# akloetgen/PARA-suite

Measured on AMD Instinct MI355X. Metric: aligned reads/sec (10Mx50bp PAR-CLIP vs hg19-size genome) on MI355X; SAM bit-exact vs own CPU restatement (parity unpinned), higher is better.
Workload: dtype u64

## Files before the change

### para-suite_amd/csrc/ps_core.h

```cpp
#pragma once
#include "ps_types.h"

namespace ps {

PS_HD uint32_t ps_popc(uint32_t x)
{
#ifdef __HIP_DEVICE_COMPILE__
    return (uint32_t)__popc(x);
#else
    return (uint32_t)__builtin_popcount(x);
#endif
}
PS_HD uint32_t pfx_mask32(int ns)
{
    return ns >= 32 ? 0xFFFFFFFFu : (ns <= 0 ? 0u : ((1u << ns) - 1u));
}

struct Blk { uint32_t x[16]; };

#ifdef __HIP_DEVICE_COMPILE__
#define PS_AS_GLOBAL(T, p) ((const __attribute__((address_space(1))) T *)(p))
#define PS_AS_GLOBAL_W(T, p) ((__attribute__((address_space(1))) T *)(p))
typedef uint32_t ps_u32x4 __attribute__((ext_vector_type(4)));
typedef uint32_t ps_u32x2 __attribute__((ext_vector_type(2)));
// ... 111 lines not shown
    blk_count4(xk, need_k ? ok_ + 1 : 0, ck);
    if (!need_k) { ck[0] = ck[1] = ck[2] = ck[3] = 0; }
    ++st.pairs;
    if (need_k && !other) ++st.same;
}
PS_HD void occ_pair1(const IndexView &ix, bwtint k, bwtint l, int c, uint32_t &ok, uint32_t &ol, LaneStats &st)
{
    int ol_ = 0, ok_ = 0;
    const uint32_t bl = blk_of(row_to_stored(ix.primary, l), ol_);
    uint32_t bk = bl;
    bool need_k = k != 0;
    if (need_k) bk = blk_of(row_to_stored(ix.primary, k - 1), ok_);
    Blk xl, xk;
    load_blk(ix.blocks, bl, xl);
    bool other = need_k && bk != bl;
    if (other) load_blk(ix.blocks, bk, xk);
    ol = blk_count1(xl, ol_ + 1, c);
    if (!need_k) ok = 0;
    else if (other) ok = blk_count1(xk, ok_ + 1, c);
    else ok = blk_count1(xl, ok_ + 1, c);
    ++st.pairs;
    if (need_k && !other) ++st.same;
}

PS_HD int read_base(const uint32_t *bases, const uint32_t *nmask, int n_reads, int r, int j)
{
    uint32_t w = bases[(size_t)(j >> 4) * n_reads + r];
    uint32_t m = nmask[(size_t)(j >> 5) * n_reads + r];
    return ((m >> (j & 31)) & 1u) ? 4 : (int)((w >> (2 * (j & 15))) & 3u);
}

PS_HD uint8_t cw_pack(int bid, bool eq) { return (uint8_t)((bid > 127 ? 127 : bid) | (eq ? 0x80 : 0)); }

struct WChain { bwtint k, l; int bid; uint32_t prev_w; };
PS_HD void wchain_init(const IndexView &ix, WChain &c) { c.k = 0; c.l = ix.seq_len; c.bid = 0; c.prev_w = 0xFFFFFFFFu; }
PS_HD void wchain_step(const IndexView &ix, WChain &c, int base, uint32_t &w_out, uint8_t &cw_out, bool first, LaneStats &st)
{
    if (base < 4) {
        uint32_t ok, ol;
        occ_pair1(ix, c.k, c.l, base, ok, ol, st);
        const bwtint l2 = L2_of(ix, base);
        c.k = l2 + ok + 1;
        c.l = l2 + ol;
    }
    if (c.k > c.l || base > 3) { c.k = 0; c.l = ix.seq_len; ++c.bid; }
    uint32_t w = width32(c.k, c.l);
    w_out = w;
    cw_out = cw_pack(c.bid, !first && w == c.prev_w);
    c.prev_w = w;
}

static const int PS_POP_TRIES = 1;
enum { M_FETCH = 0, M_POP = 1, M_EXACT = 2, M_EXPAND = 3, M_EXIT = 4, M_HIT = 5,
       M_GROW = 6 };

struct BtLane {
    int r, mode;
    bwtint k, l;
    int i, score, units, n_mm, n_gapo, n_gape, n_ins, n_del, state, ldp;
    bool have_cur;
    int best_score, max_units, n_aln, n_stack, status;
    unsigned long long best_cnt;
    unsigned long long bm0, bm1;
    uint32_t bump, free_head, iters0;
    uint32_t rn0, rn1;
    int len;
    uint32_t n_phantom;
    uint32_t cap;
    LaneStats st;
};

PS_HD int lm_ncw(int len) { return (len + 1 + 3) >> 2; }
PS_HD int lm_ncsw(int seed_len) { return seed_len > 0 ? (seed_len + 1 + 3) >> 2 : 0; }
PS_HD bool lm_nmask_in_regs(int len) { return len <= 64; }
PS_HD int lm_heads_off(int len, int seed_len) { return 4 * (lm_ncw(len) + lm_ncsw(seed_len) + ((len + 15) >> 4) + (lm_nmask_in_regs(len) ? 0 : ((len + 31) >> 5))); }
PS_HD int lm_bytes(int len, int seed_len, int n_buckets, bool wide)
{
    int n = lm_heads_off(len, seed_len) + (wide ? 0 : 2 * n_buckets);
    n = (n + 3) & ~3;
    if (((n >> 2) & 1) == 0) n += 4;
    return n;
}

static const int PS_JUMP_SLOT_WORDS = 8, PS_JUMP_MAX_LEVELS = 14;
PS_HD uint32_t jump_level_off(int d) { return 0x55555555u & ((1u << (2 * d)) - 1u); }
PS_HD size_t jump_words(int levels) { return (size_t)jump_level_off(levels) * PS_JUMP_SLOT_WORDS; }
PS_HD int jump_levels_for(bwtint seq_len) { int k = 0; while (k < PS_JUMP_MAX_LEVELS && (seq_len >> (2 * k)) >= 48) ++k; return k; }

static const int PS_CHASE_MIN2 = 16;
struct BtHot {
    const OccBlock *blocks; bwtint primary;
    const uint32_t *jump; uint32_t jump_levels;
    uint32_t skip_levels;
    uint32_t L2lo[4], L2hi;
    uint32_t s_pk[5], u_pk[5];
    uint32_t p0, p1, p2, p3;
    uint32_t inv_c_min, max_entries, pool_cap, n_reads, big_cap;
    uint32_t c_min;
    uint32_t chase;
    PS_HD int len() const { return (int)(p0 & 0xffu); }
    PS_HD int seed_len() const { return (int)((p0 >> 8) & 0xffu); }
    PS_HD int indel_end_skip() const { return (int)((p0 >> 16) & 0xffu); }
    PS_HD int max_del_occ() const { return (int)(p0 >> 24); }
    PS_HD int max_gapo() const { return (int)(p1 & 0xfu); }
    PS_HD int max_gape() const { return (int)((p1 >> 4) & 0xfu); }
    PS_HD bool mode_gape() const { return ((p1 >> 8) & 1u) != 0; }
    PS_HD bool use_seed() const { return ((p1 >> 9) & 1u) != 0; }
    PS_HD bool profile() const { return ((p1 >> 10) & 1u) != 0; }
    PS_HD bool has_big() const { return ((p1 >> 11) & 1u) != 0; }
    PS_HD int seed_units() const { return (int)((p1 >> 12) & 0xfffu); }
    PS_HD int u_tight() const { return (int)(p1 >> 24); }
    PS_HD int s_gapo_ins() const { return (int)(p2 & 0xffu); }
    PS_HD int s_gape() const { return (int)((p2 >> 8) & 0xffu); }
    PS_HD int s_gapo_del() const { return (int)((p2 >> 16) & 0xffu); }
    PS_HD int s_stop() const { return (int)(p2 >> 24); }
    PS_HD int u_gapo_ins() const { return (int)(p3 & 0xffu); }
    PS_HD int u_gape() const { return (int)((p3 >> 8) & 0xffu); }
    PS_HD int u_gapo_del() const { return (int)((p3 >> 16) & 0xffu); }
    PS_HD int n_buckets() const { return (int)(p3 >> 24); }
    PS_HD bwtint L2(int c) const
// ... 426 lines not shown
```

### para-suite_amd/csrc/ps_effort.hip

```cpp
#include <hip/hip_runtime.h>
#include "ps_core.h"
#include <stdexcept>
#include "ps_kernels.h"
#include "ps_budget.h"

namespace ps {

struct EChain {
    bwtint k, l;
    uint32_t cost_lo, cost_hi;
    int piece;
    int n_rs;
    int cl_n, cl_last;
    uint32_t cl_lo, cl_hi;
};
__device__ __forceinline__ void echain_restart(const EffortArgs &a, EChain &c, bool lo_half)
{
    c.k = 0; c.l = a.ix.seq_len; c.piece = 0; c.cl_n = 0; ++c.n_rs;
    if (lo_half) c.cost_lo += (uint32_t)a.c_restart; else c.cost_hi += (uint32_t)a.c_restart;
}
__device__ __forceinline__ void echain_step(const EffortArgs &a, EChain &c, int sym, uint32_t cw, int pos, bool lo_half, LaneStats &st)
{
    uint32_t ck[4], cl[4];
    occ_pair4(a.ix.blocks, a.ix.primary, c.k, c.l, ck, cl, st);
    if (sym < 4) {
        const uint32_t ok = sel4(ck, sym), ol = sel4(cl, sym);
        if (ok < ol) { const bwtint b = L2_of(a.ix, sym); c.k = b + ok + 1; c.l = b + ol; ++c.piece; return; }
    }
    int best = -1; uint32_t best_cost = 0xffu;
    if (c.l - c.k < (bwtint)a.w_pin) {
#pragma unroll
        for (int t = 0; t < 4; ++t) {
            const uint32_t ct = (cw >> (8 * t)) & 0xffu;
            if (t != sym && ck[t] < cl[t] && ct < best_cost) { best = t; best_cost = ct; }
        }
    }
    if (best < 0) { echain_restart(a, c, lo_half); return; }
    const int d = pos > c.cl_last ? pos - c.cl_last : c.cl_last - pos;
    if (c.cl_n > 0 && d <= 4) ++c.cl_n; else { c.cl_n = 1; c.cl_lo = c.cost_lo; c.cl_hi = c.cost_hi; }
    c.cl_last = pos;
    if (lo_half) c.cost_lo += best_cost; else c.cost_hi += best_cost;
    if (c.cl_n >= 3) {
        c.k = 0; c.l = a.ix.seq_len; c.piece = 0; c.cl_n = 0; ++c.n_rs;
        return;
    }
    const bwtint b = L2_of(a.ix, best);
    c.k = b + sel4(ck, best) + 1; c.l = b + sel4(cl, best); ++c.piece;
}

__global__ void __launch_bounds__(256, 8) k_effort(EffortArgs a)
{
    const int lane = threadIdx.x & 63;
    const bool is_b = lane >= 32;
    const int wave = (int)((blockIdx.x * blockDim.x + threadIdx.x) >> 6), n_waves = (int)((gridDim.x * blockDim.x) >> 6);
    LaneStats st = {0, 0, 0, 0, 0, 0, 0, 0};
    for (int r = wave * 32 + (lane & 31); r < a.n_reads; r += n_waves * 32) {
        const int len = a.lens ? a.lens[r] : a.len, half = len >> 1;
        EChain C = {0, a.ix.seq_len, 0, 0, 0, 0, 0, 0, 0, 0};
        uint32_t bw = 0, mw = 0;
#pragma unroll 1
        for (int i = 0; i < len; ++i) {
            const int j = is_b ? i : len - 1 - i;
            if (i == 0 || (j & 15) == (is_b ? 0 : 15)) bw = a.bases[(size_t)(j >> 4) * a.n_reads + opaque_lane(r)];
            if (i == 0 || (j & 31) == (is_b ? 0 : 31)) mw = a.nmask[(size_t)(j >> 5) * a.n_reads + opaque_lane(r)];
            const int bs = ((mw >> (j & 31)) & 1u) ? 4 : (int)((bw >> (2 * (j & 15))) & 3u);
            const int sc = bs > 3 ? 4 : 3 - bs;
            const uint32_t cws = cost_word(a.s_pk, sc);
            const uint32_t cw = is_b ? cws : __builtin_bswap32(cws);
            echain_step(a, C, is_b ? sc : bs, cw, j, j < half, st);
        }
        const uint32_t mine = C.cost_lo + C.cost_hi;
        const uint32_t tb = (uint32_t)__shfl((int)mine, lane | 32, 64), ta = mine;
        const int b_rs = __shfl(C.n_rs, lane | 32, 64), a_rs = C.n_rs;
        if (!is_b) {
            const uint32_t e = a_rs == 0 ? (b_rs == 0 && tb < ta ? tb : ta) : (b_rs == 0 ? tb : (ta > tb ? ta : tb));
            a.est[r] = (uint8_t)(e > 255u ? 255u : e);
            if (a.est_ab) a.est_ab[r] = (uint16_t)((ta > 127u ? 127u : ta) | (a_rs ? 0x80u : 0u) | ((tb > 127u ? 127u : tb) << 8) | (b_rs ? 0x8000u : 0u));
        }
    }
}

template <int G>
__global__ void __launch_bounds__(256) k_effort_model(EffortModelArgs a)
{
    const int lane = threadIdx.x & 63, u = lane & (G - 1);
    const int per_wave = 64 / G;
    const long long wave = ((long long)blockIdx.x * blockDim.x + threadIdx.x) >> 6, n_waves = ((long long)gridDim.x * blockDim.x) >> 6;
    for (long long r0 = wave * per_wave + lane / G; r0 < a.n_reads; r0 += n_waves * per_wave) {
        const int r = (int)r0;
        const int len = a.lens ? a.lens[r] : a.len;
        const int own = (a.lens && a.units_by_len) ? (int)a.units_by_len[len] : a.max_units;
        int B = (int)a.est[r] + a.u_tight;
        if (B > own) B = own;
        float w = u == 0 ? 1.f : 0.f;
        float tot = 0.f, phi_rows = a.rows;
        const int depth = len < a.depth ? len : a.depth;
        const int rem = B - u;
        const int m = rem >= 0 ? (int)(((uint32_t)rem * a.inv_c_min) >> 16) : -1;
        const int srem = a.seed_units - u;
        const bool seed_ok = srem > 0 && (int)(((uint32_t)srem * a.inv_c_min) >> 16) >= 1;
        uint32_t info = 0;
        if (u < depth) {
// ... 74 lines not shown
```

### para-suite_amd/csrc/ps_kernels.h

```cpp
#pragma once
#include <hip/hip_runtime.h>
#include "ps_types.h"
#include "ps_budget.h"

namespace ps {

static const int PS_MAX_CIGAR = 16;

struct WidthArgs {
    IndexView ix;
    int n_reads, len, seed_len, use_seed;
    const int32_t *lens;
    const uint32_t *bases; const uint32_t *nmask;
    uint32_t *w; uint32_t *cwb; uint32_t *cswb;
    KStats *stats;
};

struct EffortArgs {
    IndexView ix;
    int n_reads, len;
    const int32_t *lens;
    const uint32_t *bases; const uint32_t *nmask;
    uint32_t s_pk[5];
    int c_restart;
    uint32_t w_pin;
    uint8_t *est;
    uint16_t *est_ab;
};

struct EffortModelArgs {
    int n_reads, len;
    const int32_t *lens; const uint8_t *units_by_len;
    const uint32_t *bases; const uint32_t *nmask; const uint32_t *cwb;
    const uint8_t *est;
    uint32_t s_pk[5]; uint32_t inv_c_min;
    int max_units, u_tight, seed_units, use_seed, seed_len;
    int max_gapo, indel_end_skip, u_gapo_ins, u_gapo_del;
    int depth;
    float rows;
    int log_scale;
    uint8_t *key; float *pred;
};

struct RefineItem { int32_t read; bwtint rb; int32_t ref_shift; int32_t strand; };
struct RefineArgs {
    IndexView ix;
    int n_items, len, n_reads;
    const int32_t *lens;
    const uint32_t *bases; const uint32_t *nmask;
    const RefineItem *items;
    uint32_t *cigar; int32_t *n_cigar;
    uint8_t *zbuf; size_t z_per_block;
    int32_t *hebuf; size_t he_per_block;
// ... 34 lines not shown
```

### para-suite_amd/csrc/ps_kernels.hip

```cpp
#include <hip/hip_runtime.h>
#include <algorithm>
#include <cstdlib>
#include <stdexcept>
#include <string>
#include "ps_core.h"
#include "ps_narrow.h"
#include "ps_kernels.h"

namespace ps {

static const int PS_Q_CHUNK = 64;
#ifndef PS_BT_WAVES
#define PS_BT_WAVES 4
#endif

__device__ __forceinline__ unsigned long long wave_sum(unsigned long long v)
{
    for (int o = 32; o > 0; o >>= 1) v += __shfl_xor(v, o, 64);
    return v;
}
__device__ __forceinline__ void flush_stats(KStats *ks, const LaneStats &st)
{
    if (!ks) return;
    unsigned long long v[8] = {st.pairs, st.same, st.nodes, st.pushes, st.pops, st.lf, st.iters, st.exact};
    unsigned long long *dst = reinterpret_cast<unsigned long long *>(ks);
#pragma unroll
    for (int j = 0; j < 8; ++j) {
        unsigned long long s = wave_sum(v[j]);
        if ((threadIdx.x & 63) == 0 && s) atomicAdd(dst + j, s);
    }
}

__global__ void __launch_bounds__(256, 8) k_width(WidthArgs a)
{
    const int roles = a.use_seed ? 2 : 1;
    const bool seed_role = roles == 2 && (blockIdx.x & 1) != 0;
    const int stride = (gridDim.x / roles) * blockDim.x;
    LaneStats st = {0, 0, 0, 0, 0, 0, 0, 0};
    for (int r = (blockIdx.x / roles) * blockDim.x + threadIdx.x; r < a.n_reads; r += stride) {
        WChain C;
        wchain_init(a.ix, C);
        const int len = a.lens ? a.lens[r] : a.len, seed_len = a.seed_len;
        const bool seeded = a.use_seed && len > seed_len;
        uint32_t bw = 0, mw = 0;
        uint32_t cww = 0;
        if (!seed_role) {
#pragma unroll 1
            for (int i = 0; i < len; ++i) {
                int j = len - 1 - i;
                if (i == 0 || (j & 15) == 15) bw = a.bases[(size_t)(j >> 4) * a.n_reads + opaque_lane(r)];
                if (i == 0 || (j & 31) == 31) mw = a.nmask[(size_t)(j >> 5) * a.n_reads + opaque_lane(r)];
                int base = ((mw >> (j & 31)) & 1u) ? 4 : (int)((bw >> (2 * (j & 15))) & 3u);
                uint32_t wv; uint8_t cb;
                wchain_step(a.ix, C, base, wv, cb, i == 0, st);
                a.w[(size_t)i * a.n_reads + opaque_lane(r)] = wv;
                cww |= (uint32_t)cb << (8 * (i & 3));
                if ((i & 3) == 3) { a.cwb[(size_t)(i >> 2) * a.n_reads + opaque_lane(r)] = cww; cww = 0; }
            }
            a.w[(size_t)len * a.n_reads + opaque_lane(r)] = 0;
            cww |= (uint32_t)cw_pack(C.bid + 1, false) << (8 * (len & 3));
            a.cwb[(size_t)(len >> 2) * a.n_reads + opaque_lane(r)] = cww;
        } else if (seeded) {
#pragma unroll 1
            for (int i = 0; i < seed_len; ++i) {
                int js = seed_len - 1 - i;
                if (i == 0 || (js & 15) == 15) bw = a.bases[(size_t)(js >> 4) * a.n_reads + opaque_lane(r)];
                if (i == 0 || (js & 31) == 31) mw = a.nmask[(size_t)(js >> 5) * a.n_reads + opaque_lane(r)];
                int sbase = ((mw >> (js & 31)) & 1u) ? 4 : (int)((bw >> (2 * (js & 15))) & 3u);
                uint32_t swv; uint8_t scb;
                wchain_step(a.ix, C, sbase, swv, scb, i == 0, st);
                cww |= (uint32_t)scb << (8 * (i & 3));
                if ((i & 3) == 3) { a.cswb[(size_t)(i >> 2) * a.n_reads + opaque_lane(r)] = cww; cww = 0; }
            }
            cww |= (uint32_t)cw_pack(C.bid + 1, false) << (8 * (seed_len & 3));
            a.cswb[(size_t)(seed_len >> 2) * a.n_reads + opaque_lane(r)] = cww;
        } else if (a.use_seed) {
            for (int p = 0; p <= (seed_len >> 2); ++p) a.cswb[(size_t)p * a.n_reads + opaque_lane(r)] = 0u;
        }
    }
    flush_stats(a.stats, st);
}

__device__ __forceinline__ uint32_t pin32(uint32_t v) { return (uint32_t)__builtin_amdgcn_readfirstlane((int)v); }
__device__ __forceinline__ unsigned long long pin64(unsigned long long v)
{
    return (unsigned long long)pin32((uint32_t)v) | ((unsigned long long)pin32((uint32_t)(v >> 32)) << 32);
}
__device__ __forceinline__ void pin_hot(BtHot &h, const BtHot &k)
{
    h.blocks = reinterpret_cast<const OccBlock *>(pin64(reinterpret_cast<unsigned long long>(k.blocks)));
    h.primary = pin64(k.primary);
    h.jump = reinterpret_cast<const uint32_t *>(pin64(reinterpret_cast<unsigned long long>(k.jump))); h.jump_levels = pin32(k.jump_levels); h.skip_levels = pin32(k.skip_levels);
#pragma unroll
    for (int c = 0; c < 4; ++c) h.L2lo[c] = pin32(k.L2lo[c]);
    h.L2hi = pin32(k.L2hi);
#pragma unroll
    for (int c = 0; c < 5; ++c) { h.s_pk[c] = pin32(k.s_pk[c]); h.u_pk[c] = pin32(k.u_pk[c]); }
    h.p0 = pin32(k.p0); h.p1 = pin32(k.p1); h.p2 = pin32(k.p2); h.p3 = pin32(k.p3);
    h.c_min = pin32(k.c_min); h.chase = pin32(k.chase);
    h.inv_c_min = pin32(k.inv_c_min); h.max_entries = pin32(k.max_entries); h.pool_cap = pin32(k.pool_cap); h.n_reads = pin32(k.n_reads); h.big_cap = pin32(k.big_cap);
}

__global__ void __launch_bounds__(256) k_backtrack_wide(const BtArgs *__restrict__ ap, BtHot hk, int lm_stride)
{
    const BtArgs &a = *ap;
    BtHot h; pin_hot(h, hk);
    uint32_t *const queue = reinterpret_cast<uint32_t *>(pin64(reinterpret_cast<unsigned long long>(a.queue)));
    const uint32_t n_reads = h.n_reads, fetch_min = pin32((uint32_t)a.fetch_min), hit_min = pin32((uint32_t)a.hit_min);
    extern __shared__ __attribute__((aligned(16))) uint8_t smem[];
    const int lane_g = blockIdx.x * blockDim.x + threadIdx.x;
    BtMem m;
    bt_mem_bind(m, smem + (size_t)threadIdx.x * lm_stride, h.len(), h.seed_len());
    m.pool = reinterpret_cast<uint8_t *>(a.pool) + (size_t)lane_g * h.pool_cap * sizeof(Entry);
// ... 318 lines not shown
```

### para-suite_amd/csrc/ps_search.hip

```cpp
#include <hip/hip_runtime.h>
#include <hipcub/hipcub.hpp>
#include <algorithm>
#include <cstring>
#include <optional>
#include "ps_pipeline.h"
#include "ps_search_plan.h"
#include "ps_dev.h"
#include "ps_par.h"

namespace ps {

__global__ void k_gather_alns(const AlnRec *alns, int aln_cap, const int32_t *n_aln, const uint32_t *off, int n, AlnRec *out)
{
    for (int r = blockIdx.x * blockDim.x + threadIdx.x; r < n; r += gridDim.x * blockDim.x) {
        int m = n_aln[r]; if (m > aln_cap) m = aln_cap;
        for (int j = 0; j < m; ++j) out[off[r] + j] = alns[(size_t)r * aln_cap + j];
    }
}
__global__ void k_clip_counts(const int32_t *n_aln, int aln_cap, int n, uint32_t *out)
{
    for (int r = blockIdx.x * blockDim.x + threadIdx.x; r < n; r += gridDim.x * blockDim.x) { int m = n_aln[r]; out[r] = (uint32_t)(m > aln_cap ? aln_cap : (m < 0 ? 0 : m)); }
}

__global__ void k_order_keys(const uint8_t *est, int n, int cap, uint8_t *key)
{
    for (int r = blockIdx.x * blockDim.x + threadIdx.x; r < n; r += gridDim.x * blockDim.x) {
        const int e = est[r] > cap ? cap : est[r];
        key[r] = (uint8_t)(cap - e);
    }
}

static void search_width(Batch &b, BtArgs &a, EventPair &t)
{
    Work *wk = b.wk; const size_t n = (size_t)a.n_reads;
    uint32_t *cwb = wk->ws_get<uint32_t>("cwb", (size_t)lm_ncw(a.len) * n), *cswb = wk->ws_get<uint32_t>("cswb", (size_t)(lm_ncsw(a.md.seed_len) + 1) * n);
    a.w = wk->ws_get<uint32_t>("w", (size_t)(a.len + 1) * n); a.cwb = cwb; a.cswb = cswb;
    WidthArgs wa;
    wa.ix = a.ix; wa.n_reads = a.n_reads; wa.len = a.len; wa.lens = a.lens; wa.seed_len = a.md.seed_len; wa.use_seed = a.md.use_seed;
    wa.bases = a.bases; wa.nmask = a.nmask; wa.w = a.w; wa.cwb = cwb; wa.cswb = cswb; wa.stats = b.d_stats.p + 0;
    t.start(wk->stream); launch_width(wa, wk->stream); PS_HIP(hipGetLastError()); t.stop(wk->stream); ++b.tm.n_width_launches;
}

struct OrderBufs { const uint8_t *key = nullptr; const float *pred = nullptr; };
static void search_order(Batch &b, BtArgs &a, const SearchKnobs &kn, std::optional<EventPair> &t, OrderBufs &ob)
{
    Ctx *ctx = b.ctx; Work *wk = b.wk; hipStream_t s = wk->stream;
    const Model &md = a.md; const int n = a.n_reads;
    if (a.wide || kn.order <= 0 || n < kn.order_min || md.max_units < md.c_min) return;
    t.emplace(s);
    uint8_t *est = wk->ws_get<uint8_t>("est", (size_t)n), *key = wk->ws_get<uint8_t>("okey", (size_t)n);
    int32_t *order = wk->ws_get<int32_t>("order", (size_t)n);
    EffortArgs ea;
    ea.ix = a.ix; ea.n_reads = n; ea.len = a.len; ea.lens = a.lens; ea.bases = a.bases; ea.nmask = a.nmask; ea.est = est;
    int csum = 0;
    for (int c = 0; c < 5; ++c) ea.s_pk[c] = md.u_mm_pk[c];
    for (int sc = 0; sc < 4; ++sc) for (int tc = 0; tc < 4; ++tc) if (sc != tc) csum += md.u_mm[sc][tc];
    ea.c_restart = kn.order_restart > 0 ? kn.order_restart : std::max(1, (csum + 6) / 12);
    ea.w_pin = (uint32_t)kn.order_wpin;
    int lv = 0; while (lv < 31 && (a.ix.seq_len >> (2 * lv)) > 0) ++lv;
    ea.est_ab = ctx->want_read_iters ? wk->ws_get<uint16_t>("est_ab", (size_t)n) : nullptr;
    launch_effort(ea, s);
    if (kn.order == 2) hipLaunchKernelGGL(k_order_keys, dim3(std::min((n + 255) / 256, 4096)), dim3(256), 0, s, est, n, kn.order_cap, key);
    else {
        EffortModelArgs em;
        em.n_reads = n; em.len = a.len; em.lens = a.lens; em.units_by_len = a.units_by_len; em.bases = a.bases; em.nmask = a.nmask; em.cwb = a.cwb; em.est = est;
        for (int c = 0; c < 5; ++c) em.s_pk[c] = md.u_mm_pk[c];
        em.inv_c_min = (uint32_t)md.inv_c_min; em.max_units = md.max_units; em.u_tight = md.u_tight;
        em.seed_units = md.max_seed_diff * md.u_tight; em.use_seed = md.use_seed; em.seed_len = md.seed_len;
        em.max_gapo = md.max_gapo; em.indel_end_skip = md.indel_end_skip; em.u_gapo_ins = md.u_gapo_ins; em.u_gapo_del = md.u_gapo_del;
        em.depth = lv + 3; em.rows = (float)a.ix.seq_len; em.log_scale = kn.order_scale;
        em.key = key; em.pred = ctx->want_read_iters ? wk->ws_get<float>("pred", (size_t)n) : nullptr;
        launch_effort_model(em, s);
        ob.pred = em.pred;
    }
    launch_order_sort(key, n, wk->ws_get<uint32_t>("order_tmp", order_sort_tmp_words(n)), order, s);
    PS_HIP(hipGetLastError());
    t->stop(s);
    a.order = order; a.est = est; a.est_ab = ea.est_ab; ob.key = key;
}

static const uint8_t *upload_units_by_len(Batch &b)
{
    uint8_t *tab = b.wk->pin_get<uint8_t>("units_by_len_h", 256), *d_tab = b.wk->ws_get<uint8_t>("units_by_len", 256);
    budget_units_by_len(b.ctx->opt, tab);
    PS_HIP(hipMemcpyAsync(d_tab, tab, 256, hipMemcpyHostToDevice, b.wk->stream));
    return d_tab;
// ... 1 lines not shown

static SearchPlan search_stacks(Batch &b, BtArgs &a, const SearchKnobs &kn, int lm)
{
    Ctx *ctx = b.ctx; Work *wk = b.wk; hipStream_t s = wk->stream;
    const SearchPlan p = plan_search(a.n_reads, lm, a.pool_cap, a.wide != 0, ctx->cus, ctx->bt_blocks, kn.max_per_cu, ctx->n_big);
    a.n_lanes = p.lanes;
    a.pool = wk->ws_get<uint8_t>("pool", p.pool_bytes);
    a.heads = a.wide ? wk->ws_get<uint32_t>("heads", p.head_words) : nullptr;
    a.queue = wk->ws_get<uint32_t>("queue", 16);
    PS_HIP(hipMemsetAsync(a.queue, 0, 64, s));
    if (p.n_big) {
        a.big_cap = PS_BIG_CAP; a.n_big = p.n_big;
        a.big_pool = wk->ws_get<uint8_t>("big_pool", p.big_bytes);
        a.big_next = a.queue + 4;
        a.big_busy = wk->ws_get<uint32_t>("big_busy", a.n_big);
        PS_HIP(hipMemsetAsync(a.big_busy, 0, (size_t)a.n_big * 4, s));
    }
    return p;
}

static void run_search(Batch &b, const SearchKnobs &kn, const Model &md, int n, const uint32_t *d_bases, const uint32_t *d_nmask, const int32_t *d_lens,
                       uint32_t pool_cap, int aln_cap, AlnRec *alns, int32_t *n_aln, uint8_t *status, bool first_tier = false, const int32_t *launch_ids = nullptr)
{
    Ctx *ctx = b.ctx; Work *wk = b.wk; hipStream_t s = wk->stream;
    const int len = md.len;
    const bool wide = launch_is_wide(md, pool_cap);
    BtArgs a; std::memset(&a, 0, sizeof a);
    a.ix = ctx->ix.view; a.md = md; a.n_reads = n; a.len = len; a.lens = d_lens;
    a.bases = d_bases; a.nmask = d_nmask; a.n_bw = (len + 15) / 16; a.n_mw = (len + 31) / 32;
    a.alns = alns; a.aln_cap = aln_cap; a.n_aln = n_aln; a.status = status;
    a.pool_cap = pool_cap; a.wide = wide ? 1 : 0; a.stats = b.d_stats.p + 1; a.fetch_min = kn.fetch_min; a.hit_min = kn.hit_min;
    a.no_skip = kn.skip ? 0 : 1; a.no_chase = kn.chase ? 0 : 1; a.chase_min2 = kn.chase_min2;
    EventPair t_width; std::optional<EventPair> t_order;
    search_width(b, a, t_width);
    if (d_lens) a.units_by_len = upload_units_by_len(b);
    OrderBufs ob;
    search_order(b, a, kn, t_order, ob);
    a.cap_est = (first_tier && !wide && a.est && md.profile && kn.cap) ? 1 + kn.cap_bias : 0;
    const int lm = lm_bytes(len, md.seed_len, md.n_buckets, wide);
    const SearchPlan p = search_stacks(b, a, kn, lm);
    if (ctx->want_read_iters) { a.read_iters = wk->ws_get<uint32_t>("riters", (size_t)n * PS_RI_WORDS); PS_HIP(hipMemsetAsync(a.read_iters, 0, (size_t)n * PS_RI_WORDS * 4, s)); }
    EventPair t(s);
    if (!launch_backtrack(a, wk->ws_get<BtArgs>("btargs", 1), wk->pin_get<BtArgs>("btargs_h", 1), p.blocks, lm, s, ctx->want_kstats || ctx->want_read_iters)) throw Error("cost model outside the ranges the search kernel packs (gap/score fields must fit a byte)");
    PS_HIP(hipGetLastError());
    t.stop(s);
    const double ms = t.ms(); b.tm.ms_backtrack += ms; ++b.tm.n_backtrack_launches;
    b.tm.ms_width += t_width.ms();
    if (t_order) b.tm.ms_width += t_order->ms();
    { double t0_ = 0, t1_ = 0; t.span(ctx->ref_event, t0_, t1_); if (b.tm.n_backtrack_launches == 1) b.tm.bt_begin_ms = t0_; b.tm.bt_end_ms = t1_; }
    if (std::getenv("PS_VERBOSE")) std::fprintf(stderr, "[parasuite-hip]   backtrack launch: %d reads x %d bp, stack %u%s, %d lanes, %.1f ms\n", n, len, pool_cap, wide ? " (wide)" : "", p.lanes, ms);
    if (ctx->want_read_iters) {
        ctx->read_iters.resize((size_t)n * PS_RI_WORDS); PS_HIP(hipMemcpyAsync(ctx->read_iters.data(), a.read_iters, (size_t)n * PS_RI_WORDS * 4, hipMemcpyDeviceToHost, s));
        Ctx::LaunchOrder &lo = ctx->launch_order;
        lo.clear();
        if (a.order) {
            lo.est.resize((size_t)n); lo.key.resize((size_t)n); lo.pred.assign((size_t)n, 0.f); lo.order.resize((size_t)n); lo.ids.resize((size_t)n);
            PS_HIP(hipMemcpyAsync(lo.est.data(), a.est, (size_t)n, hipMemcpyDeviceToHost, s));
            PS_HIP(hipMemcpyAsync(lo.key.data(), ob.key, (size_t)n, hipMemcpyDeviceToHost, s));
            if (ob.pred) PS_HIP(hipMemcpyAsync(lo.pred.data(), ob.pred, (size_t)n * 4, hipMemcpyDeviceToHost, s));
            PS_HIP(hipMemcpyAsync(lo.order.data(), a.order, (size_t)n * 4, hipMemcpyDeviceToHost, s));
            for (int r = 0; r < n; ++r) lo.ids[(size_t)r] = launch_ids ? launch_ids[r] : r;
        }
        PS_HIP(hipStreamSynchronize(s));
    }
}

static void download_alns(Work *wk, int n, int aln_cap, const AlnRec *d_alns, const int32_t *d_n_aln,
// ... 318 lines not shown
```

### para-suite_amd/csrc/ps_search_plan.h

```cpp
#pragma once
#include <algorithm>
#include <cstdint>
#include <cstdlib>
#include "ps_budget.h"
#include "ps_core.h"
#include "ps_error.h"
#include "ps_model.h"

namespace ps {

struct SearchKnobs {
    int order = 1, order_min = 4096, order_restart = 0 , order_wpin = 16, order_cap = 255, order_scale = 8;
    int max_per_cu = PS_SEARCH_WAVES;
    bool cap = true; int cap_bias = 0;
    bool skip = true;
    int chase_min2 = PS_CHASE_MIN2;
    bool chase = true;
    int fetch_min = 8, hit_min = 1;
    bool collapse = false;
    int collapse_hash_bits = 64;
};
inline SearchKnobs search_knobs_from_env(int ctx_fetch_min, int ctx_hit_min)
{
    SearchKnobs k; int v = 0;
    k.fetch_min = ctx_fetch_min; k.hit_min = ctx_hit_min;
    if (env_int("PS_ORDER", v)) k.order = v;
    if (env_int("PS_ORDER_MIN", v)) k.order_min = std::max(1, v);
    if (env_int("PS_ORDER_RESTART", v)) k.order_restart = std::max(1, v);
    if (env_int("PS_ORDER_WPIN", v)) k.order_wpin = std::max(1, v);
    if (env_int("PS_ORDER_CAP", v)) k.order_cap = std::max(1, std::min(255, v));
    if (env_int("PS_ORDER_SCALE", v)) k.order_scale = std::max(1, std::min(12, v));
    if (env_int("PS_MAX_PER_CU", v)) k.max_per_cu = v;
    if (env_int("PS_CAP", v)) k.cap = v != 0;
    if (env_int("PS_CAP_BIAS", v)) k.cap_bias = std::max(0, std::min(200, v));
    if (env_int("PS_SKIP", v)) k.skip = v != 0;
    if (env_int("PS_CHASE", v)) k.chase = v != 0;
    if (env_int("PS_CHASE_MIN2", v)) k.chase_min2 = std::max(1, std::min(65, v));
    if (env_int("PS_FETCH_MIN", v)) k.fetch_min = std::max(1, v);
    if (env_int("PS_HIT_MIN", v)) k.hit_min = std::max(1, v);
    if (env_int("PS_COLLAPSE", v)) k.collapse = v != 0;
    if (env_int("PS_COLLAPSE_HASH_BITS", v)) k.collapse_hash_bits = std::max(1, std::min(64, v));
    return k;
}

struct SearchPlan { int blocks = 0, lanes = 0; size_t pool_bytes = 0, head_words = 0; uint32_t n_big = 0; size_t big_bytes = 0; };
static const uint32_t PS_BIG_CAP = 65535;
inline SearchPlan plan_search(int64_t n_reads, int lm_bytes_per_lane, uint32_t pool_cap, bool wide, int cus, int bt_blocks, int max_per_cu, int n_big)
{
    int per_cu = (int)(PS_CU_LDS / ((size_t)256 * lm_bytes_per_lane));
    if (per_cu < 1) throw Error("read length / score range too large for the per-lane LDS state");
    if (bt_blocks <= 0 && max_per_cu < 1) throw Error("PS_MAX_PER_CU must be at least 1");
    int64_t blocks = std::min<int64_t>(bt_blocks > 0 ? bt_blocks : (int64_t)cus * std::min(per_cu, max_per_cu), (n_reads + 255) / 256);
    const size_t entry = wide ? sizeof(Entry) : sizeof(Entry16), per_lane = (size_t)pool_cap * entry + (wide ? PS_MAX_BUCKETS * 4 : 0);
    const size_t max_lanes = ((size_t)(wide ? 32 : 64) << 30) / per_lane;
    if ((size_t)blocks * 256 > max_lanes) blocks = (int64_t)std::max<size_t>(1, max_lanes / 256);
    SearchPlan p;
    p.blocks = (int)blocks; p.lanes = p.blocks * 256;
    p.pool_bytes = (size_t)p.lanes * pool_cap * entry;
    p.head_words = wide ? (size_t)p.lanes * PS_MAX_BUCKETS : 0;
    if (!wide && pool_cap < PS_BIG_CAP && n_big > 0) {
        p.n_big = (uint32_t)std::min<int64_t>(n_big, std::max<int64_t>(64, n_reads));
        p.big_bytes = (size_t)p.n_big * PS_BIG_CAP * sizeof(Entry16);
    }
    return p;
}
inline SearchPlan plan_search_reserve(uint32_t pool_cap, int cus, int bt_blocks, int n_big)
{
    if (pool_cap > PS_BIG_CAP) return SearchPlan();
    return plan_search(INT32_MAX, (int)PS_SEARCH_LDS_PER_LANE, pool_cap, false, cus, bt_blocks, PS_SEARCH_WAVES, n_big);
}

inline void budget_units_by_len(const Options &o, uint8_t tab[256])
{
    for (int l = 0; l < 256; ++l) { const int u = budget_diffs(o, l) * (o.profile ? o.unit : 1); tab[l] = (uint8_t)(u > 255 ? 255 : u); }
}
// ... 3 lines not shown
```

Baseline: 9.899 million.

## Use precomputed jump table to skip first BWT steps in width and effort kernels

The width and effort prep kernels now look up the first several backward-search steps of each read in a precomputed k-mer jump table, in batched vector loads, instead of doing serial occurrence lookups per base. They fall back to the per-base BWT step loop once the table depth is used up or the interval dies. This is meant to replace dependent random occ-block fetches for the early steps with independent table loads. It adds more complex control flow and extra per-read loads, and depends on the table reproducing the exact chain widths and restart semantics.

```diff
diff --git a/para-suite_amd/csrc/ps_core.h b/para-suite_amd/csrc/ps_core.h
--- a/para-suite_amd/csrc/ps_core.h
+++ b/para-suite_amd/csrc/ps_core.h
@@ -167,24 +167,6 @@
 
 PS_HD uint8_t cw_pack(int bid, bool eq) { return (uint8_t)((bid > 127 ? 127 : bid) | (eq ? 0x80 : 0)); }
 
-struct WChain { bwtint k, l; int bid; uint32_t prev_w; };
-PS_HD void wchain_init(const IndexView &ix, WChain &c) { c.k = 0; c.l = ix.seq_len; c.bid = 0; c.prev_w = 0xFFFFFFFFu; }
-PS_HD void wchain_step(const IndexView &ix, WChain &c, int base, uint32_t &w_out, uint8_t &cw_out, bool first, LaneStats &st)
-{
-    if (base < 4) {
-        uint32_t ok, ol;
-        occ_pair1(ix, c.k, c.l, base, ok, ol, st);
-        const bwtint l2 = L2_of(ix, base);
-        c.k = l2 + ok + 1;
-        c.l = l2 + ol;
-    }
-    if (c.k > c.l || base > 3) { c.k = 0; c.l = ix.seq_len; ++c.bid; }
-    uint32_t w = width32(c.k, c.l);
-    w_out = w;
-    cw_out = cw_pack(c.bid, !first && w == c.prev_w);
-    c.prev_w = w;
-}
-
 static const int PS_POP_TRIES = 1;
 enum { M_FETCH = 0, M_POP = 1, M_EXACT = 2, M_EXPAND = 3, M_EXIT = 4, M_HIT = 5,
        M_GROW = 6 };
@@ -221,6 +203,131 @@
 PS_HD uint32_t jump_level_off(int d) { return 0x55555555u & ((1u << (2 * d)) - 1u); }
 PS_HD size_t jump_words(int levels) { return (size_t)jump_level_off(levels) * PS_JUMP_SLOT_WORDS; }
 PS_HD int jump_levels_for(bwtint seq_len) { int k = 0; while (k < PS_JUMP_MAX_LEVELS && (seq_len >> (2 * k)) >= 48) ++k; return k; }
+
+PS_HD uint32_t jump_child_word(int d, uint32_t sidx, int c) { return (jump_level_off(d) + sidx) * (uint32_t)PS_JUMP_SLOT_WORDS + 2u * (uint32_t)c; }
+PS_HD void jump_load_pair(const uint32_t *jump, uint32_t word, uint32_t &ck, uint32_t &cl)
+{
+#ifdef __HIP_DEVICE_COMPILE__
+    const ps_u32x2 v = *PS_AS_GLOBAL(ps_u32x2, reinterpret_cast<const char *>(jump) + (uint32_t)(word * 4u));
+    ck = v.x; cl = v.y;
+#else
+    ck = jump[word]; cl = jump[word + 1];
+#endif
+}
+PS_HD bool jump_child(const IndexView &ix, int d, uint32_t sidx, int c, bwtint &k, bwtint &l)
+{
+    uint32_t ck, cl;
+    jump_load_pair(ix.jump, jump_child_word(d, sidx, c), ck, cl);
+    const bwtint l2 = L2_of(ix, c);
+    k = l2 + ck + 1; l = l2 + cl;
+    return ck < cl;
+}
+PS_HD void chain_window_down(const uint32_t *bases, const uint32_t *nmask, int n_reads, int r, int j0, uint32_t &sw, uint32_t &nw)
+{
+    const int wi = j0 >> 4, mi = j0 >> 5;
+    const uint32_t bh = bases[(size_t)wi * n_reads + opaque_lane(r)], bl = wi > 0 ? bases[(size_t)(wi - 1) * n_reads + opaque_lane(r)] : 0u;
+    const uint32_t mh = nmask[(size_t)mi * n_reads + opaque_lane(r)], ml = mi > 0 ? nmask[(size_t)(mi - 1) * n_reads + opaque_lane(r)] : 0u;
+    sw = (uint32_t)(((((unsigned long long)bh << 32) | bl) << (2 * (15 - (j0 & 15)))) >> 32);
+    nw = (uint32_t)(((((unsigned long long)mh << 32) | ml) << (31 - (j0 & 31))) >> 32);
+}
+PS_HD int ps_clz32(uint32_t x) { return x ? __builtin_clz(x) : 32; }
+#ifndef PS_PREP_BATCH
+#define PS_PREP_BATCH 14
+#endif
+
+struct WChain { bwtint k, l; int bid; uint32_t prev_w; };
+PS_HD void wchain_init(const IndexView &ix, WChain &c) { c.k = 0; c.l = ix.seq_len; c.bid = 0; c.prev_w = 0xFFFFFFFFu; }
+PS_HD void wchain_step(const IndexView &ix, WChain &c, int base, uint32_t &w_out, uint8_t &cw_out, bool first, LaneStats &st)
+{
+    if (base < 4) {
+        uint32_t ok, ol;
+        occ_pair1(ix, c.k, c.l, base, ok, ol, st);
+        const bwtint l2 = L2_of(ix, base);
+        c.k = l2 + ok + 1;
+        c.l = l2 + ol;
+    }
+    if (c.k > c.l || base > 3) { c.k = 0; c.l = ix.seq_len; ++c.bid; }
+    uint32_t w = width32(c.k, c.l);
+    w_out = w;
+    cw_out = cw_pack(c.bid, !first && w == c.prev_w);
+    c.prev_w = w;
+}
+PS_HD void width_chain(const IndexView &ix, int levels, const uint32_t *bases, const uint32_t *nmask, int n_reads, int r, int n,
+                       uint32_t *w, uint32_t *cw, LaneStats &st)
+{
+    WChain C;
+    wchain_init(ix, C);
+    uint32_t cww = 0;
+    int i = 0;
+    auto emit = [&](uint32_t wv, uint8_t cb) {
+        if (w) w[(size_t)i * n_reads + opaque_lane(r)] = wv;
+        cww |= (uint32_t)cb << (8 * (i & 3));
+        if ((i & 3) == 3) { cw[(size_t)(i >> 2) * n_reads + opaque_lane(r)] = cww; cww = 0; }
+        ++i;
+    };
+    const uint32_t w_full = width32(0, ix.seq_len);
+    while (i < n) {
+        if (levels > 0) {
+            uint32_t sw, nw;
+            chain_window_down(bases, nmask, n_reads, r, n - 1 - i, sw, nw);
+            const int n_at = ps_clz32(nw);
+            int tmax = levels < n - i ? levels : n - i;
+            const bool n_stop = n_at < tmax;
+            tmax = n_stop ? n_at : tmax;
+            bool live = true;
+            uint32_t lk = 0, ll = 0;
+#pragma unroll 1
+            for (int t0 = 0; t0 < tmax && live; t0 += PS_PREP_BATCH) {
+                uint32_t ck[PS_PREP_BATCH], cl[PS_PREP_BATCH];
+#pragma unroll
+                for (int u = 0; u < PS_PREP_BATCH; ++u) {
+                    const int t = t0 + u;
+                    const uint32_t x = sw >> ((30 - 2 * t) & 31);
+                    jump_load_pair(ix.jump, t < tmax ? jump_child_word(t, x >> 2, (int)(x & 3u)) : 0u, ck[u], cl[u]);
+                }
+#pragma unroll
+                for (int u = 0; u < PS_PREP_BATCH; ++u) {
+                    if (live && t0 + u < tmax) {
+                        live = ck[u] < cl[u];
+                        if (!live) ++C.bid;
+                        const uint32_t wv = live ? cl[u] - ck[u] : w_full;
+                        lk = ck[u]; ll = cl[u];
+                        const uint8_t cb = cw_pack(C.bid, i != 0 && wv == C.prev_w);
+                        C.prev_w = wv;
+                        emit(wv, cb);
+                    }
+                }
+            }
+            if (live && n_stop) {
+                ++C.bid;
+                const uint8_t cb = cw_pack(C.bid, i != 0 && w_full == C.prev_w);
+                C.prev_w = w_full;
+                emit((uint32_t)opaque_lane((int)w_full), cb);
+                live = false;
+            }
+            if (!live || i >= n) continue;
+            const int c = (int)((sw >> (32 - 2 * levels)) & 3u);
+            const bwtint l2 = L2_of(ix, c);
+            C.k = l2 + lk + 1; C.l = l2 + ll;
+        }
+        int j = n - 1 - i;
+        uint32_t bw = bases[(size_t)(j >> 4) * n_reads + opaque_lane(r)], mw = nmask[(size_t)(j >> 5) * n_reads + opaque_lane(r)];
+#pragma unroll 1
+        for (;;) {
+            const int base = ((mw >> (j & 31)) & 1u) ? 4 : (int)((bw >> (2 * (j & 15))) & 3u);
+            uint32_t wv; uint8_t cb;
+            wchain_step(ix, C, base, wv, cb, i == 0, st);
+            emit(wv, cb);
+            if (i >= n || (levels > 0 && C.k == 0)) break;
+            j = n - 1 - i;
+            if ((j & 15) == 15) bw = bases[(size_t)(j >> 4) * n_reads + opaque_lane(r)];
+            if ((j & 31) == 31) mw = nmask[(size_t)(j >> 5) * n_reads + opaque_lane(r)];
+        }
+    }
+    if (w) w[(size_t)n * n_reads + opaque_lane(r)] = 0;
+    cww |= (uint32_t)cw_pack(C.bid + 1, false) << (8 * (n & 3));
+    cw[(size_t)(n >> 2) * n_reads + opaque_lane(r)] = cww;
+}
 
 static const int PS_CHASE_MIN2 = 16;
 struct BtHot {
diff --git a/para-suite_amd/csrc/ps_effort.hip b/para-suite_amd/csrc/ps_effort.hip
--- a/para-suite_amd/csrc/ps_effort.hip
+++ b/para-suite_amd/csrc/ps_effort.hip
@@ -6,6 +6,9 @@
 
 namespace ps {
 
+#ifndef PS_EFFORT_BATCH
+#define PS_EFFORT_BATCH 14
+#endif
 struct EChain {
     bwtint k, l;
     uint32_t cost_lo, cost_hi;
@@ -48,26 +51,84 @@
     c.k = b + sel4(ck, best) + 1; c.l = b + sel4(cl, best); ++c.piece;
 }
 
+__device__ __forceinline__ void chain_window_up_rc(const EffortArgs &a, int r, int j0, uint32_t &sw, uint32_t &nw)
+{
+    const int wi = j0 >> 4, mi = j0 >> 5, n_bw = (a.len + 15) >> 4, n_mw = (a.len + 31) >> 5;
+    const uint32_t bl = a.bases[(size_t)wi * a.n_reads + opaque_lane(r)], bh = wi + 1 < n_bw ? a.bases[(size_t)(wi + 1) * a.n_reads + opaque_lane(r)] : 0u;
+    const uint32_t ml = a.nmask[(size_t)mi * a.n_reads + opaque_lane(r)], mh = mi + 1 < n_mw ? a.nmask[(size_t)(mi + 1) * a.n_reads + opaque_lane(r)] : 0u;
+    const uint32_t up = __brev(~(uint32_t)((((unsigned long long)bh << 32) | bl) >> (2 * (j0 & 15))));
+    sw = ((up & 0x55555555u) << 1) | ((up >> 1) & 0x55555555u);
+    nw = __brev((uint32_t)((((unsigned long long)mh << 32) | ml) >> (j0 & 31)));
+}
+
 __global__ void __launch_bounds__(256, 8) k_effort(EffortArgs a)
 {
     const int lane = threadIdx.x & 63;
     const bool is_b = lane >= 32;
     const int wave = (int)((blockIdx.x * blockDim.x + threadIdx.x) >> 6), n_waves = (int)((gridDim.x * blockDim.x) >> 6);
     LaneStats st = {0, 0, 0, 0, 0, 0, 0, 0};
+    const int levels = a.ix.jump ? a.jump_levels : 0;
     for (int r = wave * 32 + (lane & 31); r < a.n_reads; r += n_waves * 32) {
         const int len = a.lens ? a.lens[r] : a.len, half = len >> 1;
         EChain C = {0, a.ix.seq_len, 0, 0, 0, 0, 0, 0, 0, 0};
-        uint32_t bw = 0, mw = 0;
+        int i = 0;
+        while (i < len) {
+            if (levels > 0) {
+                uint32_t sw, nw;
+                if (!is_b) chain_window_down(a.bases, a.nmask, a.n_reads, r, len - 1 - i, sw, nw);
+                else chain_window_up_rc(a, r, i, sw, nw);
+                const int n_at = ps_clz32(nw);
+                int tmax = levels < len - i ? levels : len - i;
+                tmax = n_at < tmax ? n_at : tmax;
+                bool live = true;
+                int t_used = 0;
+                uint32_t lk = 0, ll = 0;
 #pragma unroll 1
-        for (int i = 0; i < len; ++i) {
-            const int j = is_b ? i : len - 1 - i;
-            if (i == 0 || (j & 15) == (is_b ? 0 : 15)) bw = a.bases[(size_t)(j >> 4) * a.n_reads + opaque_lane(r)];
-            if (i == 0 || (j & 31) == (is_b ? 0 : 31)) mw = a.nmask[(size_t)(j >> 5) * a.n_reads + opaque_lane(r)];
-            const int bs = ((mw >> (j & 31)) & 1u) ? 4 : (int)((bw >> (2 * (j & 15))) & 3u);
-            const int sc = bs > 3 ? 4 : 3 - bs;
-            const uint32_t cws = cost_word(a.s_pk, sc);
-            const uint32_t cw = is_b ? cws : __builtin_bswap32(cws);
-            echain_step(a, C, is_b ? sc : bs, cw, j, j < half, st);
+                for (int t0 = 0; t0 < tmax && live; t0 += PS_EFFORT_BATCH) {
+                    uint32_t ck[PS_EFFORT_BATCH], cl[PS_EFFORT_BATCH];
+#pragma unroll
+                    for (int u = 0; u < PS_EFFORT_BATCH; ++u) {
+                        const int t = t0 + u;
+                        const uint32_t x = sw >> ((30 - 2 * t) & 31);
+                        jump_load_pair(a.ix.jump, t < tmax ? jump_child_word(t, x >> 2, (int)(x & 3u)) : 0u, ck[u], cl[u]);
+                    }
+#pragma unroll
+                    for (int u = 0; u < PS_EFFORT_BATCH; ++u) {
+                        if (live && t0 + u < tmax) {
+                            live = ck[u] < cl[u];
+                            if (live) { lk = ck[u]; ll = cl[u]; t_used = t0 + u + 1; }
+                        }
+                    }
+                }
+                i += t_used; C.piece = t_used;
+                if (i >= len) break;
+                if (t_used > 0) {
+                    const int c = (int)((sw >> (32 - 2 * t_used)) & 3u);
+                    const bwtint l2 = L2_of(a.ix, c);
+                    C.k = l2 + lk + 1; C.l = l2 + ll;
+                }
+                if (t_used < levels && !(C.l - C.k < (bwtint)a.w_pin)) {
+                    const int j = is_b ? i : len - 1 - i;
+                    echain_restart(a, C, j < half);
+                    ++i;
+                    continue;
+                }
+            }
+            int j = is_b ? i : len - 1 - i;
+            uint32_t bw = a.bases[(size_t)(j >> 4) * a.n_reads + opaque_lane(r)], mw = a.nmask[(size_t)(j >> 5) * a.n_reads + opaque_lane(r)];
+#pragma unroll 1
+            for (;;) {
+                const int bs = ((mw >> (j & 31)) & 1u) ? 4 : (int)((bw >> (2 * (j & 15))) & 3u);
+                const int sc = bs > 3 ? 4 : 3 - bs;
+                const uint32_t cws = cost_word(a.s_pk, sc);
+                const uint32_t cw = is_b ? cws : __builtin_bswap32(cws);
+                echain_step(a, C, is_b ? sc : bs, cw, j, j < half, st);
+                ++i;
+                if (i >= len || (levels > 0 && C.k == 0)) break;
+                j = is_b ? i : len - 1 - i;
+                if ((j & 15) == (is_b ? 0 : 15)) bw = a.bases[(size_t)(j >> 4) * a.n_reads + opaque_lane(r)];
+                if ((j & 31) == (is_b ? 0 : 31)) mw = a.nmask[(size_t)(j >> 5) * a.n_reads + opaque_lane(r)];
+            }
         }
         const uint32_t mine = C.cost_lo + C.cost_hi;
         const uint32_t tb = (uint32_t)__shfl((int)mine, lane | 32, 64), ta = mine;
diff --git a/para-suite_amd/csrc/ps_kernels.h b/para-suite_amd/csrc/ps_kernels.h
--- a/para-suite_amd/csrc/ps_kernels.h
+++ b/para-suite_amd/csrc/ps_kernels.h
@@ -10,6 +10,7 @@
 struct WidthArgs {
     IndexView ix;
     int n_reads, len, seed_len, use_seed;
+    int jump_levels;
     const int32_t *lens;
     const uint32_t *bases; const uint32_t *nmask;
     uint32_t *w; uint32_t *cwb; uint32_t *cswb;
@@ -19,6 +20,7 @@
 struct EffortArgs {
     IndexView ix;
     int n_reads, len;
+    int jump_levels;
     const int32_t *lens;
     const uint32_t *bases; const uint32_t *nmask;
     uint32_t s_pk[5];
diff --git a/para-suite_amd/csrc/ps_kernels.hip b/para-suite_amd/csrc/ps_kernels.hip
--- a/para-suite_amd/csrc/ps_kernels.hip
+++ b/para-suite_amd/csrc/ps_kernels.hip
@@ -19,7 +19,7 @@
     for (int o = 32; o > 0; o >>= 1) v += __shfl_xor(v, o, 64);
     return v;
 }
-__device__ __forceinline__ void flush_stats(KStats *ks, const LaneStats &st)
+__device__ __forceinline__ void flush_stats(KStats *ks, const LaneStats &st, int lane)
 {
     if (!ks) return;
     unsigned long long v[8] = {st.pairs, st.same, st.nodes, st.pushes, st.pops, st.lf, st.iters, st.exact};
@@ -27,58 +27,27 @@
 #pragma unroll
     for (int j = 0; j < 8; ++j) {
         unsigned long long s = wave_sum(v[j]);
-        if ((threadIdx.x & 63) == 0 && s) atomicAdd(dst + j, s);
-    }
-}
+        if (lane == 0 && s) atomicAdd(dst + j, s);
+    }
+}
+__device__ __forceinline__ void flush_stats(KStats *ks, const LaneStats &st) { flush_stats(ks, st, (int)(threadIdx.x & 63)); }
 
 __global__ void __launch_bounds__(256, 8) k_width(WidthArgs a)
 {
-    const int roles = a.use_seed ? 2 : 1;
-    const bool seed_role = roles == 2 && (blockIdx.x & 1) != 0;
-    const int stride = (gridDim.x / roles) * blockDim.x;
+    const int two = a.use_seed ? 1 : 0;
+    const bool seed_role = two && (blockIdx.x & 1) != 0;
+    const int stride = __builtin_amdgcn_readfirstlane((int)((gridDim.x >> two) * blockDim.x));
+    const int levels = a.ix.jump ? a.jump_levels : 0;
     LaneStats st = {0, 0, 0, 0, 0, 0, 0, 0};
-    for (int r = (blockIdx.x / roles) * blockDim.x + threadIdx.x; r < a.n_reads; r += stride) {
-        WChain C;
-        wchain_init(a.ix, C);
+    for (int r = (int)((blockIdx.x >> two) * blockDim.x + threadIdx.x); r < a.n_reads; r += stride) {
         const int len = a.lens ? a.lens[r] : a.len, seed_len = a.seed_len;
         const bool seeded = a.use_seed && len > seed_len;
-        uint32_t bw = 0, mw = 0;
-        uint32_t cww = 0;
-        if (!seed_role) {
-#pragma unroll 1
-            for (int i = 0; i < len; ++i) {
-                int j = len - 1 - i;
-                if (i == 0 || (j & 15) == 15) bw = a.bases[(size_t)(j >> 4) * a.n_reads + opaque_lane(r)];
-                if (i == 0 || (j & 31) == 31) mw = a.nmask[(size_t)(j >> 5) * a.n_reads + opaque_lane(r)];
-                int base = ((mw >> (j & 31)) & 1u) ? 4 : (int)((bw >> (2 * (j & 15))) & 3u);
-                uint32_t wv; uint8_t cb;
-                wchain_step(a.ix, C, base, wv, cb, i == 0, st);
-                a.w[(size_t)i * a.n_reads + opaque_lane(r)] = wv;
-                cww |= (uint32_t)cb << (8 * (i & 3));
-                if ((i & 3) == 3) { a.cwb[(size_t)(i >> 2) * a.n_reads + opaque_lane(r)] = cww; cww = 0; }
-            }
-            a.w[(size_t)len * a.n_reads + opaque_lane(r)] = 0;
-            cww |= (uint32_t)cw_pack(C.bid + 1, false) << (8 * (len & 3));
-            a.cwb[(size_t)(len >> 2) * a.n_reads + opaque_lane(r)] = cww;
-        } else if (seeded) {
-#pragma unroll 1
-            for (int i = 0; i < seed_len; ++i) {
-                int js = seed_len - 1 - i;
-                if (i == 0 || (js & 15) == 15) bw = a.bases[(size_t)(js >> 4) * a.n_reads + opaque_lane(r)];
-                if (i == 0 || (js & 31) == 31) mw = a.nmask[(size_t)(js >> 5) * a.n_reads + opaque_lane(r)];
-                int sbase = ((mw >> (js & 31)) & 1u) ? 4 : (int)((bw >> (2 * (js & 15))) & 3u);
-                uint32_t swv; uint8_t scb;
-                wchain_step(a.ix, C, sbase, swv, scb, i == 0, st);
-                cww |= (uint32_t)scb << (8 * (i & 3));
-                if ((i & 3) == 3) { a.cswb[(size_t)(i >> 2) * a.n_reads + opaque_lane(r)] = cww; cww = 0; }
-            }
-            cww |= (uint32_t)cw_pack(C.bid + 1, false) << (8 * (seed_len & 3));
-            a.cswb[(size_t)(seed_len >> 2) * a.n_reads + opaque_lane(r)] = cww;
-        } else if (a.use_seed) {
+        if (!seed_role || seeded) width_chain(a.ix, levels, a.bases, a.nmask, a.n_reads, r, seed_role ? seed_len : len, seed_role ? nullptr : a.w, seed_role ? a.cswb : a.cwb, st);
+        else {
             for (int p = 0; p <= (seed_len >> 2); ++p) a.cswb[(size_t)p * a.n_reads + opaque_lane(r)] = 0u;
         }
     }
-    flush_stats(a.stats, st);
+    flush_stats(a.stats, st, (int)__builtin_amdgcn_mbcnt_hi(~0u, __builtin_amdgcn_mbcnt_lo(~0u, 0u)));
 }
 
 __device__ __forceinline__ uint32_t pin32(uint32_t v) { return (uint32_t)__builtin_amdgcn_readfirstlane((int)v); }
diff --git a/para-suite_amd/csrc/ps_search.hip b/para-suite_amd/csrc/ps_search.hip
--- a/para-suite_amd/csrc/ps_search.hip
+++ b/para-suite_amd/csrc/ps_search.hip
@@ -30,13 +30,13 @@
     }
 }
 
-static void search_width(Batch &b, BtArgs &a, EventPair &t)
+static void search_width(Batch &b, BtArgs &a, const SearchKnobs &kn, EventPair &t)
 {
     Work *wk = b.wk; const size_t n = (size_t)a.n_reads;
     uint32_t *cwb = wk->ws_get<uint32_t>("cwb", (size_t)lm_ncw(a.len) * n), *cswb = wk->ws_get<uint32_t>("cswb", (size_t)(lm_ncsw(a.md.seed_len) + 1) * n);
     a.w = wk->ws_get<uint32_t>("w", (size_t)(a.len + 1) * n); a.cwb = cwb; a.cswb = cswb;
     WidthArgs wa;
-    wa.ix = a.ix; wa.n_reads = a.n_reads; wa.len = a.len; wa.lens = a.lens; wa.seed_len = a.md.seed_len; wa.use_seed = a.md.use_seed;
+    wa.ix = a.ix; wa.jump_levels = prep_jump_levels(kn, a.ix, b.ctx->want_kstats); wa.n_reads = a.n_reads; wa.len = a.len; wa.lens = a.lens; wa.seed_len = a.md.seed_len; wa.use_seed = a.md.use_seed;
     wa.bases = a.bases; wa.nmask = a.nmask; wa.w = a.w; wa.cwb = cwb; wa.cswb = cswb; wa.stats = b.d_stats.p + 0;
     t.start(wk->stream); launch_width(wa, wk->stream); PS_HIP(hipGetLastError()); t.stop(wk->stream); ++b.tm.n_width_launches;
 }
@@ -51,7 +51,7 @@
     uint8_t *est = wk->ws_get<uint8_t>("est", (size_t)n), *key = wk->ws_get<uint8_t>("okey", (size_t)n);
     int32_t *order = wk->ws_get<int32_t>("order", (size_t)n);
     EffortArgs ea;
-    ea.ix = a.ix; ea.n_reads = n; ea.len = a.len; ea.lens = a.lens; ea.bases = a.bases; ea.nmask = a.nmask; ea.est = est;
+    ea.ix = a.ix; ea.jump_levels = prep_jump_levels(kn, a.ix, false); ea.n_reads = n; ea.len = a.len; ea.lens = a.lens; ea.bases = a.bases; ea.nmask = a.nmask; ea.est = est;
     int csum = 0;
     for (int c = 0; c < 5; ++c) ea.s_pk[c] = md.u_mm_pk[c];
     for (int sc = 0; sc < 4; ++sc) for (int tc = 0; tc < 4; ++tc) if (sc != tc) csum += md.u_mm[sc][tc];
@@ -119,7 +119,7 @@
     a.pool_cap = pool_cap; a.wide = wide ? 1 : 0; a.stats = b.d_stats.p + 1; a.fetch_min = kn.fetch_min; a.hit_min = kn.hit_min;
     a.no_skip = kn.skip ? 0 : 1; a.no_chase = kn.chase ? 0 : 1; a.chase_min2 = kn.chase_min2;
     EventPair t_width; std::optional<EventPair> t_order;
-    search_width(b, a, t_width);
+    search_width(b, a, kn, t_width);
     if (d_lens) a.units_by_len = upload_units_by_len(b);
     OrderBufs ob;
     search_order(b, a, kn, t_order, ob);
diff --git a/para-suite_amd/csrc/ps_search_plan.h b/para-suite_amd/csrc/ps_search_plan.h
--- a/para-suite_amd/csrc/ps_search_plan.h
+++ b/para-suite_amd/csrc/ps_search_plan.h
@@ -16,6 +16,7 @@
     bool skip = true;
     int chase_min2 = PS_CHASE_MIN2;
     bool chase = true;
+    bool prep_jump = true;
     int fetch_min = 8, hit_min = 1;
     bool collapse = false;
     int collapse_hash_bits = 64;
@@ -36,11 +37,19 @@
     if (env_int("PS_SKIP", v)) k.skip = v != 0;
     if (env_int("PS_CHASE", v)) k.chase = v != 0;
     if (env_int("PS_CHASE_MIN2", v)) k.chase_min2 = std::max(1, std::min(65, v));
+    if (env_int("PS_PREP_JUMP", v)) k.prep_jump = v != 0;
+    if (env_int("PS_JUMP", v) && v == 0) k.prep_jump = false;
     if (env_int("PS_FETCH_MIN", v)) k.fetch_min = std::max(1, v);
     if (env_int("PS_HIT_MIN", v)) k.hit_min = std::max(1, v);
     if (env_int("PS_COLLAPSE", v)) k.collapse = v != 0;
     if (env_int("PS_COLLAPSE_HASH_BITS", v)) k.collapse_hash_bits = std::max(1, std::min(64, v));
     return k;
+}
+
+inline int prep_jump_levels(const SearchKnobs &k, const IndexView &ix, bool counting)
+{
+    if (!k.prep_jump || counting || !ix.jump) return 0;
+    return std::min(ix.jump_levels, (int)PS_JUMP_MAX_LEVELS);
 }
 
 struct SearchPlan { int blocks = 0, lanes = 0; size_t pool_bytes = 0, head_words = 0; uint32_t n_big = 0; size_t big_bytes = 0; };
```

Result: slower. 9.782 million (-1.2%).
